# wanxinjin/Learning-from-Sparse-Demonstrations

Measured on AMD Instinct MI355X. Metric: CPDP outer iterations/sec (batch trajectories), higher is better.
Workload: dtype f32; 1 GPU; Quadrotor (JinEnv, initCost_Polynomial, beta time-warp) CPDP, n_grid(horizon) 50 x 4 RK4 steps, batch 4096 per GPU, Nesterov mu 0.9, cold-start OC solve every iteration; BASELINE configs[2]: random initial-guess seeds, one theta and optimizer state per seed, lr 0.01; mode=independent, batch_per_gpu=4096, outer_iters_per_run=50, n_grid=50, steps_per_grid=4, aux_substeps=0, oc_iters_max=7, aux_intervals_accepted_above_rtol=0

## Files before the change

### learning-from-sparse-demonstrations_amd/csrc/cpdp_common.h

```cpp
#pragma once


#include <type_traits>
#if defined(LFSD_EMU)
#include "simt_emu.h"
#define LFSD_LAMBDA_INLINE
#define LFSD_HD
#else
#include <hip/hip_runtime.h>
#define LFSD_DEV __device__ __forceinline__
#define LFSD_HD __host__ __device__
#define LFSD_LAMBDA_INLINE __attribute__((always_inline))
#endif

#ifndef LFSD_COARSE_START
#define LFSD_COARSE_START 1
#endif
#ifndef LFSD_LEAN_TC
#define LFSD_LEAN_TC 2
#endif
#ifndef LFSD_MS
#define LFSD_MS 1
#endif
#ifndef LFSD_COARSE_TIME
#define LFSD_COARSE_TIME 4
#endif
#ifndef LFSD_BW_SMALL
#define LFSD_BW_SMALL 1
#endif
#ifndef LFSD_RIC_PAIR_STAGE
#define LFSD_RIC_PAIR_STAGE 1
#endif

#if defined(LFSD_EMU)
#define LFSD_ROW_FENCE()
#define LFSD_SCHED_FENCE64(T)
#else
#define LFSD_ROW_FENCE() __builtin_amdgcn_sched_barrier(0)
#define LFSD_SCHED_FENCE64(T) do { if constexpr (sizeof(T) == 8) __builtin_amdgcn_sched_barrier(0); } while (0)
#endif

#if defined(LFSD_EMU)
#define LFSD_WAVE_SYNC() __syncthreads()
#else
#define LFSD_WAVE_SYNC()                                            \
  do {                                                              \
    __builtin_amdgcn_fence(__ATOMIC_RELEASE, "workgroup", "local"); \
    __builtin_amdgcn_wave_barrier();                                \
    __builtin_amdgcn_fence(__ATOMIC_ACQUIRE, "workgroup", "local"); \
  } while (0)
#endif

#if defined(LFSD_EMU)
#define LFSD_STAGE_SYNC() __syncthreads()
#else
#define LFSD_STAGE_SYNC() LFSD_WAVE_SYNC()
#endif
#if defined(LFSD_EMU)
#define LFSD_STAGE_SYNC_GEN() __syncthreads()
#else
#define LFSD_STAGE_SYNC_GEN() LFSD_WAVE_SYNC()
#endif

namespace lfsd {

constexpr double kMuUp = 3.1623;
constexpr double kMuDown = 0.31623;
constexpr int kMuHold = 1;
constexpr double kMuStageFracNewton = 0.001;
constexpr double kHamSwitch = 0.3;

constexpr double kCoarseSwitch = 1e-3;
constexpr int kLeanTcS = 1;
constexpr int kLeanTcIters = 3;
constexpr int kLeanTcMin = 12;
constexpr int kLeanTcGrace = 2;
constexpr int kCoarseMinGrid = 40;
constexpr int kMsMinGrid = 40;
constexpr int kCoarseTimeS = 2;
constexpr int kCoarseTimeMin = 20;
constexpr double kCoarseExitMu = 1e-2;
constexpr int kCsAhead = 3;
constexpr int kWideMaxBatch = 1536;

// ... 403 lines not shown
    matmul<n>(A, P, W);
#pragma unroll
    for (int i = 0; i < n * n; ++i) P[i] = -W[i];
#pragma unroll
    for (int i = 0; i < n; ++i) P[i * n + i] += ck[k];
  }
  matmul<n>(A, P, W);
#pragma unroll
  for (int i = 0; i < n * n; ++i) E[i] = -W[i];
#pragma unroll
  for (int i = 0; i < n; ++i) E[i * n + i] += T(1);
  for (int it = 0; it < sq; ++it) {
    matmul<n>(E, P, W);
#pragma unroll
    for (int i = 0; i < n * n; ++i) P[i] = T(0.5) * (P[i] + W[i]);
    matmul<n>(E, E, W);
#pragma unroll
    for (int i = 0; i < n * n; ++i) E[i] = W[i];
  }
  matmul<n>(E, P, W);
#pragma unroll
  for (int i = 0; i < n * n; ++i) P2[i] = T(0.5) * (P[i] + W[i]);
}
template <int Q> constexpr bool sub_ok() { return Q == 1 || Q == 2 || Q == 4; }
#if defined(LFSD_EMU)
template <int Q, typename T> inline T sub_bcast(T v, int k) {
  static_assert(sub_ok<Q>(), "sub-group of 1, 2 or 4 lanes");
  if (Q == 1) return v;
  static T sb[EMU_MAXT];
  const int l = threadIdx.x;
  sb[l] = v;
  __syncthreads();
  const T r = sb[(l & ~(Q - 1)) | k];
  __syncthreads();
  return r;
}
#else
template <int CTRL> LFSD_DEV float dpp_mov(float v) {
  return __builtin_bit_cast(float, __builtin_amdgcn_mov_dpp(__builtin_bit_cast(int, v), CTRL, 0xf, 0xf, true));
}
template <int CTRL> LFSD_DEV double dpp_mov(double v) {
  const unsigned long long u = __builtin_bit_cast(unsigned long long, v);
  const int lo = __builtin_amdgcn_mov_dpp((int)(unsigned)u, CTRL, 0xf, 0xf, true);
  const int hi = __builtin_amdgcn_mov_dpp((int)(unsigned)(u >> 32), CTRL, 0xf, 0xf, true);
  return __builtin_bit_cast(double, ((unsigned long long)(unsigned)hi << 32) | (unsigned long long)(unsigned)lo);
}
template <int Q, typename T> LFSD_DEV T sub_bcast(T v, int k) {
  static_assert(sub_ok<Q>(), "sub-group of 1, 2 or 4 lanes");
  if constexpr (Q == 1) return v;
  else if constexpr (Q == 2) return k == 0 ? dpp_mov<0xA0>(v) : dpp_mov<0xF5>(v);
  else return k == 0 ? dpp_mov<0x00>(v) : (k == 1 ? dpp_mov<0x55>(v) : (k == 2 ? dpp_mov<0xAA>(v) : dpp_mov<0xFF>(v)));
}
#endif
template <int n> constexpr int sub_lanes() { return n <= 1 ? 1 : (n == 2 ? 2 : 4); }
template <int n, int Q, typename T> LFSD_DEV void matmul_rows(const T* Arow, const T* Brow, T* Wrow) {
#pragma unroll
  for (int j = 0; j < n; ++j) Wrow[j] = T(0);
#pragma unroll
  for (int k = 0; k < n; ++k) {
#pragma unroll
    for (int j = 0; j < n; ++j) Wrow[j] += Arow[k] * sub_bcast<Q>(Brow[j], k);
  }
}
template <int n, int Q, typename T> LFSD_DEV void phi1_neg_rows(const T* Mrow, int a, int sq, T sc, T* P, T* P2) {
  T A[n], E[n], W[n];
  const T ck[10] = {T(1), T(1) / T(2), T(1) / T(6), T(1) / T(24), T(1) / T(120), T(1) / T(720), T(1) / T(5040),
                    T(1) / T(40320), T(1) / T(362880), T(1) / T(3628800)};
  constexpr int DEG = PhiDeg<T>::v;
#pragma unroll
  for (int j = 0; j < n; ++j) { A[j] = Mrow[j] * sc; P[j] = (j == a) ? ck[DEG] : T(0); }
#pragma unroll
  for (int k = DEG - 1; k >= 0; --k) {
    matmul_rows<n, Q>(A, P, W);
#pragma unroll
    for (int j = 0; j < n; ++j) P[j] = ((j == a) ? ck[k] : T(0)) - W[j];
  }
  matmul_rows<n, Q>(A, P, W);
#pragma unroll
  for (int j = 0; j < n; ++j) E[j] = ((j == a) ? T(1) : T(0)) - W[j];
  for (int it = 0; it < sq; ++it) {
    matmul_rows<n, Q>(E, P, W);
#pragma unroll
    for (int j = 0; j < n; ++j) P[j] = T(0.5) * (P[j] + W[j]);
    matmul_rows<n, Q>(E, E, W);
#pragma unroll
    for (int j = 0; j < n; ++j) E[j] = W[j];
  }
  matmul_rows<n, Q>(E, P, W);
#pragma unroll
  for (int j = 0; j < n; ++j) P2[j] = T(0.5) * (P[j] + W[j]);
}
template <int n, typename T> LFSD_DEV void matvec(const T* A, const T* v, T* y) {
#pragma unroll
  for (int i = 0; i < n; ++i) {
    T s = T(0);
#pragma unroll
    for (int k = 0; k < n; ++k) s += A[i * n + k] * v[k];
    y[i] = s;
  }
}

}
```

### learning-from-sparse-demonstrations_amd/csrc/cpdp_oc.h

```cpp
#pragma once
#include "cpdp_common.h"

namespace lfsd {

template <typename T> struct OcArgs {
  int batch, n_grid, steps_per_grid, max_iter;
  const T* ini_state;
  const T* horizon;
  const T* auxvar;
  const T* consts;
  int const_stride;
  const T* u_init;
  T* state_grid;
  T* control_grid;
  T* costate_grid;
  T* cost;
  int* iters;
  int* status;
  T* ws;
  long long ws_stride;
  T tol;
  int exact_after;
  int it_start;
  int max_iter_total;
// ... 1252 lines not shown

  LFSD_DEV void costate_sweep_mf(int cur, bool live, T& gnorm) {
    static_assert(G == 16 && NX <= 16 && NEXT <= 1, "16-lane groups, at most one column beyond 16");
    T* ldsME = lds + Lay::LDS_M;  T* ldsLam = lds + Lay::LDS_LAM;  T* ldsRed = lds + Lay::LDS_RED;
    T lam[NX], xk[NX], uk[NU];
    {
      const T* xN = xbp(cur) + N * NX;
#pragma unroll
      for (int i = 0; i < NX; ++i) xk[i] = xN[i];
      M::final_grad(tk(N), xk, e, c, lam);
      if (lane == 0 && live) {
#pragma unroll
        for (int i = 0; i < NX; ++i) lam_out[N * NX + i] = lam[i];
      }
    }
    T gl_max = T(0);
    T m[NX], mq = T(0), me = T(0), mN[NX], mqN = T(0), meN = T(0);
    mf_load_stage(cur, N - 1, m, mq, me, xk, uk);
    for (int k = N - 1; k >= 0; --k) {
      if (NEXT) { if (lane <= NX) ldsME[lane] = me; }
      if (k > 0) { mf_load_stage(cur, k - 1, mN, mqN, meN, xk, uk); LFSD_ISSUE_FENCE(); }
      T gl = mq;
#pragma unroll
      for (int i = 0; i < NX; ++i) gl += m[i] * lam[i];
      if (lane < NX) ldsLam[lane] = gl;
      else if (lane < NCL) gl_max = t_max(gl_max, t_abs(gl));
      __syncthreads();
      if (NEXT) {
        T gl_e = ldsME[NX];
#pragma unroll
        for (int kk = 0; kk < NX; ++kk) gl_e += ldsME[kk] * lam[kk];
        gl_max = t_max(gl_max, (lane == NX) ? t_abs(gl_e) : T(0));
      }
#pragma unroll
      for (int i = 0; i < NX; ++i) lam[i] = ldsLam[i];
      if (lane == 0 && live) {
#pragma unroll
        for (int i = 0; i < NX; ++i) lam_out[k * NX + i] = lam[i];
      }
      __syncthreads();
#pragma unroll
      for (int i = 0; i < NX; ++i) m[i] = mN[i];
      mq = mqN; me = meN;
    }
    ldsRed[lane] = gl_max;
    __syncthreads();
    gnorm = T(0);
#pragma unroll
    for (int a = 0; a < NUL; ++a) gnorm = t_max(gnorm, ldsRed[NX + a]);
    __syncthreads();
  }

  static constexpr int ZC = Lay::ZC, LIVE = Lay::LIVE, LX = NX - Lay::ZC, MS = Lay::MS_ELEMS, LIVEP = Lay::LIVEP;
  LFSD_DEV T rollout_sens_sc(int cur, int nxt, T alpha, bool gains) {
    using V = pk2<T>;
    T x[NX], u[NU], J = T(0);
#pragma unroll
    for (int i = 0; i < NX; ++i) x[i] = x0[i];
    const int c0 = ZC + 2 * lane, c1 = c0 + 1;
    T ubN[NU], xbN[NX], KN[NX * NU], kN[NU];
    auto load_ctl = [&](int k_) LFSD_LAMBDA_INLINE {
      const T* ubk = ubp(cur) + k_ * NU;
#pragma unroll
      for (int a = 0; a < NU; ++a) ubN[a] = ubk[a];
      if (gains) {
        const T* xbk = xbp(cur) + k_ * NX;
        const T* Kk = Kws + (long long)k_ * NX * NU;
        const T* kk = kws + k_ * NU;
#pragma unroll
        for (int i = 0; i < NX; ++i) xbN[i] = xbk[i];
#pragma unroll
        for (int i = 0; i < NX * NU; ++i) KN[i] = Kk[i];
#pragma unroll
        for (int a = 0; a < NU; ++a) kN[a] = kk[a];
      }
    };
    load_ctl(0);
    for (int k = 0; k < N; ++k) {
#pragma unroll
      for (int a = 0; a < NU; ++a) u[a] = ubN[a];
      if (gains) {
#pragma unroll
        for (int a = 0; a < NU; ++a) u[a] += alpha * kN[a];
#pragma unroll
        for (int i = 0; i < NX; ++i) {
          const T dx = x[i] - xbN[i];
#pragma unroll
          for (int a = 0; a < NU; ++a) u[a] += KN[i * NU + a] * dx;
        }
      }
      if (k + 1 < N) { load_ctl(k + 1); LFSD_ISSUE_FENCE(); }
      if (lane == 0) {
#pragma unroll
        for (int i = 0; i < NX; ++i) xbp(nxt)[k * NX + i] = x[i];
#pragma unroll
        for (int a = 0; a < NU; ++a) ubp(nxt)[k * NU + a] = u[a];
      }
      V m[NX], du[NU], mq = V(T(0));
      T q = T(0), qz[ZC ? ZC : 1];
#pragma unroll
      for (int i = 0; i < ZC; ++i) qz[i] = T(0);
#pragma unroll
      for (int i = 0; i < NX; ++i) m[i] = mk2<T>((c0 == i) ? T(1) : T(0), (c1 == i) ? T(1) : T(0));
#pragma unroll
      for (int a = 0; a < NU; ++a) du[a] = mk2<T>((c0 == NX + a) ? T(1) : T(0), (c1 == NX + a) ? T(1) : T(0));
      const T t = tk(k);
// ... 29 lines not shown
      for (int i = 0; i < NX; ++i) m[i] = T(0);
      mq = T(0);
    }
    qzl = (lane >= LX && lane < NX) ? Mk[(NX + 1) * LIVEP + (lane - LX)] : T(0);
    const T* xp = xbp(cur) + k * NX;  const T* up = ubp(cur) + k * NU;
#pragma unroll
    for (int i = 0; i < NX; ++i) xk[i] = xp[i];
#pragma unroll
    for (int a = 0; a < NU; ++a) uk[a] = up[a];
  }
  LFSD_DEV bool backward_sc(int cur, int mode, T mu, bool live, T& gnorm, T& dV1, T& dV2, T& dmin) {
    static_assert(!Lay::sc_ok || (G == 16 && LIVE <= 16 && ZC <= NU && NX <= 16), "structural sweep: 16-lane groups");
    T* ldsV = lds + Lay::LDS_V;  T* ldsK = lds + Lay::LDS_K;
    T* ldsQux = lds + Lay::LDS_QUX;  T* ldsQuu = lds + Lay::LDS_QUU;  T* ldsQu = lds + Lay::LDS_QU;
    T* ldsVx = lds + Lay::LDS_VX;  T* ldsLam = lds + Lay::LDS_LAM;  T* ldsRed = lds + Lay::LDS_RED;
    constexpr bool MM = sizeof(T) == 4;
    constexpr bool VXR = MM;
    T* ldsMl = lds + Lay::LDS_M;
    T* ldsYZ = MM ? lds + Lay::LDS_M : yz64;
    const bool has_v = lane < NX;
    const bool st_zc = lane >= LX && lane < NX;
    const int sv = has_v ? (lane < LX ? ZC + lane : lane - LX) : 0;
    const int zi = st_zc ? lane - LX : 0;
    const bool ctl = lane >= LX && lane < LIVE;
    T Vx[NX], lam[NX], vcol[NX], xk[NX], uk[NU];
    bool ok = true;
    T gl_max = T(0);
    dV1 = T(0); dV2 = T(0); dmin = T(0);
    {
      const T* xN = xbp(cur) + N * NX;
#pragma unroll
      for (int i = 0; i < NX; ++i) xk[i] = xN[i];
      M::final_grad(tk(N), xk, e, c, Vx);
      T ox[NX], oe[NP];
#pragma unroll
      for (int i = 0; i < NX; ++i) { ox[i] = (has_v && sv == i) ? T(1) : T(0); lam[i] = Vx[i]; }
#pragma unroll
      for (int i = 0; i < NP; ++i) oe[i] = T(0);
      M::final_hess_mul(tk(N), xk, e, c, ox, oe, vcol);
      if (lane == 0) {
#pragma unroll
        for (int i = 0; i < NX; ++i) { ldsVx[i] = Vx[i]; ldsLam[i] = lam[i]; }
        if (live) {
#pragma unroll
          for (int i = 0; i < NX; ++i) lam_out[N * NX + i] = lam[i];
        }
      }
      if (!MM && has_v) {
#pragma unroll
        for (int i = 0; i < NX; ++i) ldsV[sv * NX + i] = vcol[i];
      }
    }
    __syncthreads();
    T m[NX], mq = T(0), qzl = T(0);
    sc_load_stage(cur, N - 1, m, mq, qzl, xk, uk);
    for (int k = N - 1; k >= 0; --k) {
      {
#pragma unroll
        for (int a = 0; a < NU; ++a) pin(uk[a]);
#pragma unroll
        for (int i = 0; i < NX; ++i) pin(xk[i]);
        pin(mq); pin(qzl);
      }
      typename std::conditional<MM, f32x16, T[16]>::type acc;
      T yn[NX];
      if constexpr (!MM) {
        if (lane < LIVE) {
#pragma unroll
          for (int i = 0; i < NX; ++i) ldsMl[lane * NX + i] = m[i];
        }
        LFSD_STAGE_SYNC();
        T rowb[2][NX];
#pragma unroll
        for (int kk = 0; kk < NX; ++kk) rowb[0][kk] = ldsV[kk];
#pragma unroll
        for (int r = 0; r < NX + LIVE; ++r) {
          const T* nxt = (r + 1 < NX) ? ldsV + (r + 1) * NX : ldsMl + (r + 1 - NX) * NX;
          if (r + 1 < NX + LIVE) {
#pragma unroll
            for (int kk = 0; kk < NX; ++kk) rowb[(r + 1) & 1][kk] = nxt[kk];
          }
          T sacc = T(0);
          if (r < NX) {
#pragma unroll
            for (int kk = 0; kk < NX; ++kk) sacc += rowb[r & 1][kk] * m[kk];
          } else {
#pragma unroll
            for (int kk = 0; kk < NX; ++kk) sacc += rowb[r & 1][kk] * yn[kk];
          }
          pin(sacc);
          if (r < NX) yn[r] = sacc; else acc[r - NX] = sacc;
          LFSD_ROW_FENCE();
        }
      }
      if constexpr (MM) {
#pragma unroll
      for (int r = 0; r < 16; ++r) acc[r] = 0.f;
#pragma unroll
      for (int kk = 0; kk < NX; ++kk) mfma4b(vcol[kk], m[kk], acc);
      }
      T hx[NX], hu[NU];
      {
        T ox[NX], ou[NU], ls[NX];
        const T HL = (mode == 1) ? T(1) : T(0);
#pragma unroll
        for (int i = 0; i < NX; ++i) { ox[i] = (has_v && sv == i) ? T(1) : T(0); ls[i] = HL * (VXR ? lam[i] : ldsLam[i]); }
#pragma unroll
        for (int a = 0; a < NU; ++a) ou[a] = (lane == LX + a) ? T(1) : T(0);
        M::ham_hess_mul(tk(k), xk, uk, ls, e, c, ox, ou, hx, hu);
      }
      if constexpr (MM) {
        tile_transpose(acc);
#pragma unroll
        for (int s_ = 0; s_ < NX; ++s_) yn[s_] = acc[s_ < ZC ? LX + s_ : s_ - ZC];
      }
      if (lane < LIVE) {
#pragma unroll
        for (int z = 0; z < ZC; ++z) ldsYZ[lane * ZC + z] = yn[z];
      }
      if constexpr (MM) {
#pragma unroll
        for (int r = 0; r < 16; ++r) acc[r] = 0.f;
#pragma unroll
        for (int kk = 0; kk < NX; ++kk) mfma4b(m[kk], yn[kk], acc);
      }
      T Qg = mq, gl = mq;
      if constexpr (VXR) {
#pragma unroll
        for (int i = 0; i < NX; ++i) { Qg += m[i] * Vx[i]; gl += m[i] * lam[i]; }
      } else {
        T vxl[NX], lml[NX];
#pragma unroll
        for (int i = 0; i < NX; ++i) { vxl[i] = ldsVx[i]; lml[i] = ldsLam[i]; }
#pragma unroll
        for (int i = 0; i < NX; ++i) { Qg += m[i] * vxl[i]; gl += m[i] * lml[i]; }
      }
      if constexpr (MM) tile_transpose(acc);
      LFSD_STAGE_SYNC();
      T Qcol[NX], mu_rows[NU], Quxj[NU];
#pragma unroll
      for (int a = 0; a < NU; ++a) mu_rows[a] = acc[LX + a] + dgrid * hu[a];
      T gzv[LIVE];
#pragma unroll
      for (int j = 0; j < LIVE; ++j) gzv[j] = ldsYZ[j * ZC + zi];
      T Vx_z = ldsVx[zi], lam_z = ldsLam[zi];
#pragma unroll
      for (int j = 0; j < LIVE; ++j) pin(gzv[j]);
      pin(Vx_z); pin(lam_z);
#pragma unroll
      for (int j = 0; j < LX; ++j)
        Qcol[ZC + j] = st_zc ? gzv[j] : acc[j] + dgrid * hx[ZC + j];
#pragma unroll
      for (int z = 0; z < ZC; ++z) Qcol[z] = st_zc ? vcol[z] + dgrid * hx[z] : yn[z];
#pragma unroll
      for (int a = 0; a < NU; ++a) Quxj[a] = st_zc ? gzv[LX + a] : mu_rows[a];
      const T Qg_v = st_zc ? qzl + Vx_z : Qg;
      const T gl_v = st_zc ? qzl + lam_z : gl;
      if (has_v) {
#pragma unroll
        for (int a = 0; a < NU; ++a) ldsQux[sv * NU + a] = Quxj[a];
      }
      if (ctl) {
        const int b = lane - LX;
#pragma unroll
        for (int a = 0; a < NU; ++a) ldsQuu[b * NU + a] = mu_rows[a];
        ldsQu[b] = Qg;
        gl_max = t_max(gl_max, t_abs(gl));
      }
      LFSD_STAGE_SYNC();
      T Quu0[NU * NU], Lc[NU * NU], Qu[NU], kff[NU], Kj[NU], t1[NU];
#pragma unroll
      for (int a = 0; a < NU; ++a) {
        Qu[a] = ldsQu[a];
#pragma unroll
        for (int b = 0; b < NU; ++b) Quu0[a * NU + b] = T(0.5) * (ldsQuu[b * NU + a] + ldsQuu[a * NU + b]);
      }
#pragma unroll
      for (int i = 0; i < NU * NU; ++i) Lc[i] = Quu0[i];
#pragma unroll
      for (int a = 0; a < NU; ++a) Lc[a * NU + a] += mu;
      if (ok) ok = chol_factor<NU>(Lc, dmin); else { T dd = T(0); chol_factor<NU>(Lc, dd); }
      {
#pragma unroll
        for (int a = 0; a < NU; ++a) Quu0[a * NU + a] += mu;
      }
#pragma unroll
      for (int a = 0; a < NU; ++a) { kff[a] = -Qu[a]; Kj[a] = -Quxj[a]; }
      chol_solve<NU>(Lc, kff);
      chol_solve<NU>(Lc, Kj);
      T qk[NU];
      matvec<NU>(Quu0, kff, qk);
#pragma unroll
      for (int a = 0; a < NU; ++a) { dV1 += kff[a] * Qu[a]; dV2 += T(0.5) * kff[a] * qk[a]; }
      T Vxj = Qg_v;
#pragma unroll
      for (int a = 0; a < NU; ++a) { Vxj += Kj[a] * (qk[a] + Qu[a]); Vxj += Quxj[a] * kff[a]; }
      if (has_v) {
#pragma unroll
        for (int a = 0; a < NU; ++a) ldsK[sv * NU + a] = Kj[a];
        ldsVx[sv] = Vxj;
        ldsLam[sv] = gl_v;
        if (live) {
          T* Kout = Kws + ((long long)k * NX + sv) * NU;
#pragma unroll
          for (int a = 0; a < NU; ++a) Kout[a] = Kj[a];
        }
      }
      if (lane == 0 && live) {
#pragma unroll
        for (int a = 0; a < NU; ++a) kws[k * NU + a] = kff[a];
      }
      LFSD_STAGE_SYNC();
      matvec<NU>(Quu0, Kj, t1);
#pragma unroll
      for (int a = 0; a < NU; ++a) t1[a] += Quxj[a];
#pragma unroll
      for (int i = 0; i < NX; ++i) {
        T sacc = Qcol[i];
#pragma unroll
        for (int a = 0; a < NU; ++a) { sacc += ldsK[i * NU + a] * t1[a]; sacc += ldsQux[i * NU + a] * Kj[a]; }
        vcol[i] = sacc;
        if (VXR) { Vx[i] = ldsVx[i]; lam[i] = ldsLam[i]; }
      }
      if (lane == 0 && live) {
#pragma unroll
        for (int i = 0; i < NX; ++i) lam_out[k * NX + i] = VXR ? lam[i] : ldsLam[i];
      }
      if (has_v) {
#pragma unroll
        for (int i = 0; i < NX; ++i) ldsV[sv * NX + i] = vcol[i];
      }
      LFSD_STAGE_SYNC();
      {
        T vt[NX];
#pragma unroll
        for (int i = 0; i < NX; ++i) vt[i] = ldsV[i * NX + sv];
#pragma unroll
        for (int i = 0; i < NX; ++i) pin(vt[i]);
#pragma unroll
        for (int i = 0; i < NX; ++i) vcol[i] = has_v ? T(0.5) * (vcol[i] + vt[i]) : T(0);
      }
      LFSD_STAGE_SYNC();
      if (!MM && has_v) {
#pragma unroll
        for (int i = 0; i < NX; ++i) ldsV[sv * NX + i] = vcol[i];
      }
      if (k > 0) sc_load_stage(cur, k - 1, m, mq, qzl, xk, uk);
    }
    ldsRed[lane] = gl_max;
    __syncthreads();
    gnorm = T(0);
#pragma unroll
    for (int a = 0; a < NU; ++a) gnorm = t_max(gnorm, ldsRed[LX + a]);
    __syncthreads();
    if (!t_finite(gnorm) || !t_finite(dV1) || !t_finite(dV2)) ok = false;
    return ok;
  }
  LFSD_DEV void costate_sweep_sc(int cur, bool live, T& gnorm) {
    T* ldsLam = lds + Lay::LDS_LAM;  T* ldsRed = lds + Lay::LDS_RED;
    const bool has_v = lane < NX, st_zc = lane >= LX && lane < NX, ctl = lane >= LX && lane < LIVE;
    const int sv = has_v ? (lane < LX ? ZC + lane : lane - LX) : 0;
    const int zi = st_zc ? lane - LX : 0;
    T lam[NX], xk[NX], uk[NU];
    {
      const T* xN = xbp(cur) + N * NX;
#pragma unroll
      for (int i = 0; i < NX; ++i) xk[i] = xN[i];
      M::final_grad(tk(N), xk, e, c, lam);
      if (lane == 0) {
#pragma unroll
        for (int i = 0; i < NX; ++i) ldsLam[i] = lam[i];
        if (live) {
#pragma unroll
          for (int i = 0; i < NX; ++i) lam_out[N * NX + i] = lam[i];
        }
      }
    }
    __syncthreads();
    T gl_max = T(0);
    T m[NX], mq = T(0), qzl = T(0), mN[NX], mqN = T(0), qzN = T(0);
    sc_load_stage(cur, N - 1, m, mq, qzl, xk, uk);
    for (int k = N - 1; k >= 0; --k) {
      if (k > 0) { sc_load_stage(cur, k - 1, mN, mqN, qzN, xk, uk); LFSD_ISSUE_FENCE(); }
      T gl = mq;
#pragma unroll
      for (int i = 0; i < NX; ++i) gl += m[i] * lam[i];
      if (ctl) gl_max = t_max(gl_max, t_abs(gl));
      T lam_z = ldsLam[zi];
      pin(lam_z);
      const T glz = qzl + lam_z;
      __syncthreads();
      if (has_v) ldsLam[sv] = st_zc ? glz : gl;
      __syncthreads();
#pragma unroll
      for (int i = 0; i < NX; ++i) lam[i] = ldsLam[i];
      if (lane == 0 && live) {
#pragma unroll
        for (int i = 0; i < NX; ++i) lam_out[k * NX + i] = lam[i];
      }
      __syncthreads();
#pragma unroll
      for (int i = 0; i < NX; ++i) m[i] = mN[i];
      mq = mqN; qzl = qzN;
    }
    ldsRed[lane] = gl_max;
    __syncthreads();
    gnorm = T(0);
#pragma unroll
    for (int a = 0; a < NU; ++a) gnorm = t_max(gnorm, ldsRed[LX + a]);
    __syncthreads();
  }

  LFSD_DEV int linesearch(int cur, T J, T dV1, T dV2, T& alpha_out, T& Jmin, bool& flat_full) {
    T* ldsRed = lds + Lay::LDS_RED;
    T alpha = T(0);
    if (lane < NALPHA) { alpha = T(1); for (int i = 0; i < lane; ++i) alpha *= T(0.5); }
    T x[NX], u[NU], Ja = T(0), dummy = T(0);
#pragma unroll
    for (int i = 0; i < NX; ++i) x[i] = x0[i];
    for (int k = 0; k < N; ++k) {
      control(cur, k, x, alpha, true, u);
      T q = T(0);
      const T t = tk(k);
      for (int s = 0; s < S; ++s) rk4_step<false>(t, x, q, u, x, dummy, u);
      Ja += q;
    }
    Ja += M::final_cost(tk(N), x, e, c);
    ldsRed[lane] = Ja;
    __syncthreads();
    int ia = -1;
    Jmin = J;
    T a = T(1);
    alpha_out = T(0);
    const T flat = T(8) * Eps<T>::v() * t_abs(J);
    flat_full = t_finite(ldsRed[0]) && t_abs(ldsRed[0] - J) <= T(64) * Eps<T>::v() * t_abs(J);
    for (int l = 0; l < NALPHA; ++l) {
      const T Jl = ldsRed[l];
      const T expected = -(a * dV1 + a * a * dV2);
      const bool okl = t_finite(Jl) && ((J - Jl) >= T(1e-4) * expected - flat) && (Jl < J);
      if (okl && ia < 0) { ia = l; alpha_out = a; }
      if (t_finite(Jl)) Jmin = t_min(Jmin, Jl);
      a *= T(0.5);
    }
    __syncthreads();
    return ia;
  }
};

template <class M, typename T, bool EXACT, bool BND = false, int W = 1> struct OcWide : OcSolver<M, T, 64, EXACT, BND> {
  using Base = OcSolver<M, T, 64, EXACT, BND>;
  using Lay = OcLayout<M>;
  static constexpr int NX = M::NX, NU = M::NU, NP = M::NP, NXU = NX + NU;
  static constexpr int NAL = 16;
  static constexpr int NW = W, PSTRIDE = 64 * W;
  int wave = 0;
  LFSD_DEV int pitem() const { return W == 1 ? lane : wave * 64 + lane; }
  using Base::lane; using Base::N; using Base::S; using Base::e; using Base::c; using Base::x0; using Base::xb; using Base::ub; using Base::xbp; using Base::ubp; using Base::Mwp;
  using Base::Mws; using Base::Hws; using Base::lds; using Base::xa; using Base::ua; using Base::lam_out; using Base::DT;

  LFSD_DEV T rollout_alphas(int cur, bool gains, T& alpha) {
    alpha = T(0);
    if (lane < NAL) { alpha = T(1); for (int i = 0; i < lane; ++i) alpha *= T(0.5); }
    T x[NX], u[NU], Ja = T(0), dummy = T(0);
// ... 1520 lines not shown
```

### learning-from-sparse-demonstrations_amd/isa_check.py

```python
import re

_FUNC = re.compile(r"^([A-Za-z_][\w$.]*):")
_BLOCK = re.compile(r"^(\.LBB\d+_\d+):")
_EXECZ = re.compile(r"^\s+s_cbranch_execz\s+(\.LBB\d+_\d+)")
_EXECNZ = re.compile(r"^\s+s_cbranch_execnz\s+(\.LBB\d+_\d+)")
_RESTORE = re.compile(r"^(s_or_b64\s+exec,\s*exec,|s_or_saveexec_b64|s_andn2_saveexec_b64|s_xor_b64\s+exec,\s*exec,)")
_SPILL_STORE = re.compile(r"^(v_accvgpr_write_b32\s+a\d+,\s*v\d+|scratch_store_\w+\s.*Folded Spill)")
_SPILL_LOAD = re.compile(r"^(v_accvgpr_read_b32\s+(v\d+),\s*a\d+|scratch_load_(\w+)\s+(v\d+|v\[\d+:\d+\]),.*Folded Reload)")
_VREG = re.compile(r"\bv(\d+)\b|\bv\[(\d+):(\d+)\]")
_EXEC_WRITE = re.compile(r"^s_\w*saveexec|^s_\w+\s+exec\b|^s_mov_b64\s+exec|^s_cmov\w*\s+exec")


def _regs(text):
    out = set()
    for m in _VREG.finditer(text):
        if m.group(1) is not None:
            out.add(int(m.group(1)))
        else:
            out.update(range(int(m.group(2)), int(m.group(3)) + 1))
    return out


def _operands(instr):
    body = instr.split(";")[0]
# ... 31 lines not shown
        else:
            continue
        j, stores, loads, restore_at = i + 1, [], [], -1
        while j < n and (not lines[j].strip() or lines[j].strip().startswith(";") or (label.startswith("behind") and _BLOCK.match(lines[j]))):
            if _BLOCK.match(lines[j]) and _BLOCK.match(lines[j]).group(1) in targets:
                break
            j += 1
        if j < n and _BLOCK.match(lines[j]) and label.startswith("behind"):
            continue
        while j < n:
            t = lines[j].strip()
            if not t or t.startswith(";"):
                j += 1
                continue
            if t.startswith(".L") or t.startswith(("s_branch", "s_cbranch", "s_endpgm", "s_setpc")):
                break
            if _RESTORE.match(t):
                restore_at = j
                break
            if _EXEC_WRITE.match(t):
                break
            if _SPILL_STORE.match(t):
                stores.append((j + 1, t))
            else:
                ml = _SPILL_LOAD.match(t)
                if ml:
                    loads.append((j + 1, t, _regs(ml.group(2) or ml.group(4))))
            j += 1
        if restore_at < 0:
            continue
        for at, t in stores:
            hazards.append({"function": func, "block": label, "line": at, "kind": "spill", "instr": t})
        for at, t, regs in loads:
            pending, k = set(regs), restore_at + 1
            bad = False
            while k < n and pending:
                u = lines[k].strip()
                if not u or u.startswith(";"):
                    k += 1
                    continue
                if u.startswith(".L") or u.startswith(("s_branch", "s_cbranch", "s_endpgm", "s_setpc")):
                    break
                w, r = _operands(u)
                if r & pending:
                    bad = True
                    break
                pending -= w
                k += 1
            if bad:
                hazards.append({"function": func, "block": label, "line": at, "kind": "reload", "instr": t})
    return hazards


def summary(asm_text):
    targets = set(m.group(1) for m in (_EXECZ.match(ln) for ln in asm_text.split("\n")) if m)
    nfunc = sum(1 for ln in asm_text.split("\n") if ln.startswith(".Lfunc_end"))
    return {"functions": nfunc, "join_blocks": len(targets)}
```

### learning-from-sparse-demonstrations_amd/runtime.py

```python
import ctypes
import os
import shutil
import subprocess

import torch

PKG_DIR = os.path.dirname(os.path.abspath(__file__))
CSRC_DIR = os.path.join(PKG_DIR, "csrc")
GEN_DIR = os.path.join(CSRC_DIR, "gen")
BUILD_DIR = os.path.join(CSRC_DIR, "build")
INCLUDE_DIR = os.path.join(os.path.dirname(PKG_DIR), "include")

LFSD_F32, LFSD_F64 = 0, 1
STATUS = {1: "converged", 2: "stalled", 3: "maxiter", 4: "failed"}
OPT_METHODS = {"Vanilla": 0, "Nesterov": 1, "Adam": 2, "Nadam": 3, "AMSGrad": 4, "LM": 5}
MAPPINGS = {"auto": 0, "lockstep": 1, "wide": 2}


class LfsdError(RuntimeError):
    pass


class _ModelInfo(ctypes.Structure):
    _fields_ = [("abi_version", ctypes.c_int), ("n_state", ctypes.c_int), ("n_control", ctypes.c_int),
# ... 18 lines not shown
            return cand
    raise LfsdError("hipcc not found: the HIP model library cannot be built")


def library_path(model_hash):
    return os.path.join(BUILD_DIR, "liblfsd_%s.so" % model_hash)


def header_path(model_hash):
    return os.path.join(GEN_DIR, "%s.h" % model_hash)


def write_header(spec, force=False):
    from . import codegen
    os.makedirs(GEN_DIR, exist_ok=True)
    hp = header_path(spec.hash())
    if force or not os.path.exists(hp):
        src = codegen.emit_header(spec)
        tmp = hp + ".tmp%d" % os.getpid()
        with open(tmp, "w") as f:
            f.write(src)
        os.replace(tmp, hp)
    return hp


def _hipcc_flags(spec, extra=()):
    g = lanes_for(spec.n, spec.m, spec.p)
    return [find_hipcc(), "-x", "hip", "--offload-arch=gfx950", "-std=c++17", "-O3", "-fPIC",
            "-fno-signed-zeros", "-fvisibility=hidden",
            "-DLFSD_G=%d" % g, '-DLFSD_MODEL_HEADER="gen/%s.h"' % spec.hash(), "-I" + CSRC_DIR] + list(extra)


TUNED_CAPI = ()
TUNED_RICCATI = ()
TUNED_CUBIC = ()
UNITS = ("capi", "riccati", "cubic")


def hipcc_commands(spec, out, extra=(), extra_capi=TUNED_CAPI, extra_riccati=TUNED_RICCATI, extra_cubic=TUNED_CUBIC):
    flags = _hipcc_flags(spec, extra) + ["-fno-slp-vectorize"]
    o1, o2, o3 = out + ".capi.o", out + ".riccati.o", out + ".cubic.o"
    return ([flags + ["-c", "-DLFSD_SPLIT_RICCATI", os.path.join(CSRC_DIR, "lfsd_capi.cpp"), "-o", o1] + list(extra_capi),
             flags + ["-c", os.path.join(CSRC_DIR, "lfsd_riccati.cpp"), "-o", o2] + list(extra_riccati),
             flags + ["-c", os.path.join(CSRC_DIR, "lfsd_cubic.cpp"), "-o", o3] + list(extra_cubic),
             [find_hipcc(), "--offload-arch=gfx950", "-shared", "-fPIC", o1, o2, o3, "-o", out]], [o1, o2, o3])


KERNEL_SOURCES = ("cpdp_kernels.h", "cpdp_common.h", "cpdp_oc.h", "cpdp_aux.h", "cpdp_opt.h", "cpdp_rows.h", "cpdp_spline.h", "cpdp_sample.h", "cpdp_lm.h", "cpdp_groups.h", "cpdp_aux_sweeps.inc", "lfsd_capi.cpp",
                  "lfsd_internal.h", "lfsd_riccati.inc", "lfsd_riccati.cpp", "lfsd_cubic.inc", "lfsd_cubic.cpp")


SCHEDULE_ALTERNATES = ((), ("-mllvm", "-amdgpu-sched-strategy=max-ilp"), ("-mllvm", "-amdgpu-sched-strategy=max-memory-clause"),
                       ("-mllvm", "-amdgpu-use-amdgpu-trackers"), ("-mllvm", "-greedy-reverse-local-assignment"))
ISA_CHECK_VERSION = 3


def isa_record_path(lib_path):
    return lib_path + ".isa.json"


def isa_record_clean(lib_path):
    import json
    try:
        rec = json.load(open(isa_record_path(lib_path)))
    except (OSError, ValueError):
        return False
    units = rec.get("units", {})
    return rec.get("isa_check") == ISA_CHECK_VERSION and set(units) == set(UNITS) and all(u.get("hazards") == 0 for u in units.values()) \
        and rec.get("sha256") == _sha256(lib_path)


def _sha256(path):
    import hashlib
    h = hashlib.sha256()
    with open(path, "rb") as f:
        for chunk in iter(lambda: f.read(1 << 20), b""):
            h.update(chunk)
    return h.hexdigest()


def _checked_build(spec, out, extra=(), verbose=False, what="model"):
    import json, shutil, tempfile
    from . import isa_check
    os.makedirs(BUILD_DIR, exist_ok=True)
    work = tempfile.mkdtemp(prefix="obj%d_" % os.getpid(), dir=BUILD_DIR)
    try:
        tmp = os.path.join(work, "lib.so")
        record = {"isa_check": ISA_CHECK_VERSION, "units": {}}
        objs = []
        for ui, unit in enumerate(UNITS):
            tuned = (TUNED_CAPI, TUNED_RICCATI, TUNED_CUBIC)[ui]
            tried, built = [], False
            for alt in SCHEDULE_ALTERNATES:
                kw = {"extra_" + unit: tuple(tuned) + tuple(alt)}
                cmds, obj_paths = hipcc_commands(spec, tmp, list(extra), **kw)
                cmd = cmds[ui] + ["-save-temps=obj"]
                if verbose:
                    print(" ".join(cmd))
                for f in os.listdir(work):
                    if f.endswith(".s"):
                        os.remove(os.path.join(work, f))
                r = subprocess.run(cmd, cwd=CSRC_DIR, capture_output=True, text=True)
                if r.returncode != 0:
                    if alt:
                        tried.append({"flags": list(alt), "error": r.stderr[-300:]})
                        continue
                    raise LfsdError("hipcc failed for %s %s:\n%s\n%s" % (what, spec.name, r.stdout[-4000:], r.stderr[-4000:]))
                asm = [f for f in os.listdir(work) if f.endswith("gfx950.s")]
                if len(asm) != 1:
                    raise LfsdError("no device assembly to check for %s %s (%s): %s" % (what, spec.name, unit, sorted(os.listdir(work))))
                text = open(os.path.join(work, asm[0])).read()
                hz = isa_check.find_exec_hazards(text)
                if hz:
                    tried.append({"flags": list(alt), "hazards": len(hz), "first": hz[0]})
                    if verbose:
                        print("isa_check: %d spill(s) before an exec restore in %s (%s, flags %s): %s" % (len(hz), spec.name, unit, list(alt), hz[0]))
                    continue
                record["units"][unit] = dict(isa_check.summary(text), flags=list(tuned) + list(alt), hazards=0, rejected=tried)
                objs.append(obj_paths[ui])
                built = True
                break
            if not built:
                raise LfsdError("every build of %s %s (%s) has VGPR spills before an exec restore (lfsd_amd/isa_check.py): %s"
                                % (what, spec.name, unit, tried))
        link = hipcc_commands(spec, tmp, list(extra))[0][-1]
        r = subprocess.run(link, cwd=CSRC_DIR, capture_output=True, text=True)
        if r.returncode != 0:
            raise LfsdError("link failed for %s %s:\n%s" % (what, spec.name, r.stderr[-3000:]))
        record["sha256"] = _sha256(tmp)
        with open(isa_record_path(out) + ".tmp%d" % os.getpid(), "w") as f:
            json.dump(record, f, indent=1, sort_keys=True, default=str)
        os.replace(tmp, out)
        os.replace(isa_record_path(out) + ".tmp%d" % os.getpid(), isa_record_path(out))
        return record
    finally:
        shutil.rmtree(work, ignore_errors=True)


def build_library(spec, force=False, verbose=False):
    os.makedirs(BUILD_DIR, exist_ok=True)
    out = library_path(spec.hash())
    write_header(spec, force=force)
    deps = [header_path(spec.hash()), os.path.join(INCLUDE_DIR, "lfsd_cpdp.h")] + \
        [os.path.join(CSRC_DIR, f) for f in KERNEL_SOURCES]
    if not force and os.path.exists(out) and all(os.path.getmtime(out) >= os.path.getmtime(d) for d in deps) and isa_record_clean(out):
        return out
    _checked_build(spec, out, verbose=verbose)
    return out


def variant_library_path(spec, tag):
    return os.path.join(BUILD_DIR, "ab_%s_%s.so" % (spec.hash(), tag))


def build_variant_library(spec, tag, flags):
    write_header(spec)
    out = variant_library_path(spec, tag)
    deps = [header_path(spec.hash())] + [os.path.join(CSRC_DIR, f) for f in KERNEL_SOURCES]
    if os.path.exists(out) and all(os.path.getmtime(out) >= os.path.getmtime(p) for p in deps) and isa_record_clean(out):
        return out
    _checked_build(spec, out, extra=list(flags), what="variant %s of model" % tag)
    return out


PLAIN_SCHEDULE = ("-DLFSD_LEAN_TC=1", "-DLFSD_COARSE_START=0", "-DLFSD_COARSE_TIME=1", "-DLFSD_MS=0")
GPU_TIER_VARIANTS = (("quadrotor", 50, "nocoarse", ("-DLFSD_COARSE_START=0",)),
                     ("quadrotor", 50, "plain", PLAIN_SCHEDULE), ("cartpole", 40, "plain", PLAIN_SCHEDULE),
                     ("rocket", 40, "plain", PLAIN_SCHEDULE), ("robotarm", 50, "plain", PLAIN_SCHEDULE),
                     ("quadrotor", 50, "ricpair0", ("-DLFSD_RIC_PAIR_STAGE=0",)))


def build_gpu_tier_variants(verbose=False):
    from concurrent.futures import ThreadPoolExecutor
    from . import models
    built = {}
    with ThreadPoolExecutor(max_workers=max(1, min(4, (os.cpu_count() or 2) // 2))) as pool:
        futs = {}
        for kind, n_grid, tag, flags in GPU_TIER_VARIANTS:
            oc = models.ZOO[kind](n_grid=n_grid)[0]
            futs[(kind, tag)] = pool.submit(build_variant_library, oc.model_spec(), tag, flags)
        for (kind, tag), fut in futs.items():
            try:
                built[(kind, tag)] = fut.result()
                if verbose:
                    print("variant", kind, tag, built[(kind, tag)])
            except Exception as exc:
                print("WARNING: test variant %s/%s not built: %s" % (kind, tag, str(exc)[:300]))
    return built


_DT = {torch.float32: LFSD_F32, torch.float64: LFSD_F64}


class ModelLibrary:

    EXPORTS = ("lfsd_get_model_info", "lfsd_interface_dim", "lfsd_const_default", "lfsd_coc_workspace_bytes", "lfsd_coc_solve",
               "lfsd_aux_solve", "lfsd_aux_riccati", "lfsd_aux_forward", "lfsd_optimizer_step", "lfsd_lookahead",
               "lfsd_stop_compact", "lfsd_gather_rows", "lfsd_scatter_rows", "lfsd_grid_curvature", "lfsd_aux_solve_cubic",
               "lfsd_aux_riccati_cubic", "lfsd_aux_forward_cubic", "lfsd_sample_grid", "lfsd_waypoint_vjp",
               "lfsd_optimizer_step_rows", "lfsd_lookahead_rows", "lfsd_trace_append", "lfsd_normal_matrix", "lfsd_lm_step",
               "lfsd_group_reduce")

    def __init__(self, path):
        if not os.path.exists(path):
            raise LfsdError("model library %s does not exist (build it with __graft_entry__.build() or "
                            "COCSys.compile())" % path)
        self.path = path
        self.lib = ctypes.CDLL(path)
        for sym in self.EXPORTS:
            if not hasattr(self.lib, sym):
                raise LfsdError("%s does not export %s" % (path, sym))
        L = self.lib
        vp, ci, cd = ctypes.c_void_p, ctypes.c_int, ctypes.c_double
        L.lfsd_get_model_info.argtypes = [ctypes.POINTER(_ModelInfo)]
        L.lfsd_const_default.argtypes = [ci]
        L.lfsd_const_default.restype = cd
        L.lfsd_coc_workspace_bytes.argtypes = [ci, ci, ci, ci, ci, ci]
        L.lfsd_coc_workspace_bytes.restype = ctypes.c_size_t
        L.lfsd_coc_solve.argtypes = [ci, ci, ci, ci, vp, vp, vp, vp, ci, vp, vp, vp, vp, vp, vp, cd, vp, vp, vp, vp, vp, vp, ci, cd, ci,
                                     ci, vp, ctypes.c_size_t, vp]
        L.lfsd_aux_solve.argtypes = [ci, ci, ci, vp, vp, vp, ci, vp, vp, vp, vp, ci, ci, vp, vp, vp, vp, vp, vp, vp,
                                     ci, cd, vp, vp, ci, vp]
# ... 526 lines not shown
```

Baseline: 960,200 trajectory outer-iterations/s.

## Replace LDS exchanges in the OC backward Riccati sweep with DPP row broadcasts

In the sensitivity/costate backward sweep, when a group is one 16-lane row and T is f32, per-stage LDS writes, stage syncs and reads of Quu, Qu, K, Qux, Vx and lambda are replaced by DPP row_newbcast broadcasts and inline v_fmac_f32_dpp asm. The final gradient-norm reduction also moves from LDS to row broadcasts. The aim is to remove LDS traffic and barriers on the serial per-stage critical path. In exchange it adds hand-written DPP asm with an s_nop settle, and an ISA checker that rejects builds placing DPP reads too close to a writer, which could force a fallback schedule.

Result: faster. 987,900 trajectory outer-iterations/s (median of 6 runs) (+2.9%).

```diff
diff --git a/learning-from-sparse-demonstrations_amd/csrc/cpdp_common.h b/learning-from-sparse-demonstrations_amd/csrc/cpdp_common.h
--- a/learning-from-sparse-demonstrations_amd/csrc/cpdp_common.h
+++ b/learning-from-sparse-demonstrations_amd/csrc/cpdp_common.h
@@ -2,6 +2,7 @@
 
 
 #include <type_traits>
+#include <utility>
 #if defined(LFSD_EMU)
 #include "simt_emu.h"
 #define LFSD_LAMBDA_INLINE
@@ -30,6 +31,9 @@
 #endif
 #ifndef LFSD_RIC_PAIR_STAGE
 #define LFSD_RIC_PAIR_STAGE 1
+#endif
+#ifndef LFSD_OC_DPP_XCHG
+#define LFSD_OC_DPP_XCHG 1
 #endif
 
 #if defined(LFSD_EMU)
@@ -539,6 +543,48 @@
   else return k == 0 ? dpp_mov<0x00>(v) : (k == 1 ? dpp_mov<0x55>(v) : (k == 2 ? dpp_mov<0xAA>(v) : dpp_mov<0xFF>(v)));
 }
 #endif
+constexpr bool row_xchg_ok(int lanes) { return lanes == 16; }
+#if defined(LFSD_EMU)
+template <typename T> inline T row_bcast(T v, int k) {
+  static T sb[EMU_MAXT];
+  const int l = threadIdx.x;
+  sb[l] = v;
+  __syncthreads();
+  const T r = sb[(l & ~15) | k];
+  __syncthreads();
+  return r;
+}
+#else
+LFSD_DEV float row_bcast(float v, int k) {
+  switch (k) {
+    case 0: return dpp_mov<0x150>(v);   case 1: return dpp_mov<0x151>(v);   case 2: return dpp_mov<0x152>(v);   case 3: return dpp_mov<0x153>(v);
+    case 4: return dpp_mov<0x154>(v);   case 5: return dpp_mov<0x155>(v);   case 6: return dpp_mov<0x156>(v);   case 7: return dpp_mov<0x157>(v);
+    case 8: return dpp_mov<0x158>(v);   case 9: return dpp_mov<0x159>(v);   case 10: return dpp_mov<0x15A>(v);  case 11: return dpp_mov<0x15B>(v);
+    case 12: return dpp_mov<0x15C>(v);  case 13: return dpp_mov<0x15D>(v);  case 14: return dpp_mov<0x15E>(v);  default: return dpp_mov<0x15F>(v);
+  }
+}
+#endif
+#if defined(LFSD_EMU)
+inline void dpp_settle() {}
+template <int K> inline void fmac2_row_bcast(float& acc, float a, float wa, float b, float wb) {
+  acc += row_bcast(a, K) * wa;
+  acc += row_bcast(b, K) * wb;
+}
+#else
+LFSD_DEV void dpp_settle() { asm volatile("s_nop 4"); }
+template <int K> LFSD_DEV void fmac2_row_bcast(float& acc, float a, float wa, float b, float wb) {
+  static_assert(K >= 0 && K < 16, "lane of the row");
+  asm volatile("v_fmac_f32_dpp %0, %1, %2 row_newbcast:%5 row_mask:0xf bank_mask:0xf bound_ctrl:1\n\t"
+               "v_fmac_f32_dpp %0, %3, %4 row_newbcast:%5 row_mask:0xf bank_mask:0xf bound_ctrl:1"
+               : "+v"(acc) : "v"(a), "v"(wa), "v"(b), "v"(wb), "n"(K));
+}
+#endif
+template <typename T> LFSD_DEV T row_max(T v, int first, int n) {
+  T r = T(0);
+#pragma unroll
+  for (int a = 0; a < n; ++a) r = t_max(r, row_bcast(v, first + a));
+  return r;
+}
 template <int n> constexpr int sub_lanes() { return n <= 1 ? 1 : (n == 2 ? 2 : 4); }
 template <int n, int Q, typename T> LFSD_DEV void matmul_rows(const T* Arow, const T* Brow, T* Wrow) {
 #pragma unroll
diff --git a/learning-from-sparse-demonstrations_amd/csrc/cpdp_oc.h b/learning-from-sparse-demonstrations_amd/csrc/cpdp_oc.h
--- a/learning-from-sparse-demonstrations_amd/csrc/cpdp_oc.h
+++ b/learning-from-sparse-demonstrations_amd/csrc/cpdp_oc.h
@@ -1328,6 +1328,16 @@
   }
 
   static constexpr int ZC = Lay::ZC, LIVE = Lay::LIVE, LX = NX - Lay::ZC, MS = Lay::MS_ELEMS, LIVEP = Lay::LIVEP;
+  static constexpr bool XD = (LFSD_OC_DPP_XCHG != 0) && sizeof(T) == 4 && row_xchg_ok(G);
+  static constexpr int sc_lane(int i) { return i < ZC ? LX + i : i - ZC; }
+  template <int I> LFSD_DEV void sc_vrow(T& sacc, const T* Kj, const T* t1, const T* Quxj) const {
+#pragma unroll
+    for (int a = 0; a < NU; ++a) fmac2_row_bcast<sc_lane(I)>(sacc, Kj[a], t1[a], Quxj[a], Kj[a]);
+  }
+  template <int... I> LFSD_DEV void sc_vrows(T* vcol, const T* Kj, const T* t1, const T* Quxj, std::integer_sequence<int, I...>) const {
+    dpp_settle();
+    (sc_vrow<I>(vcol[I], Kj, t1, Quxj), ...);
+  }
   LFSD_DEV T rollout_sens_sc(int cur, int nxt, T alpha, bool gains) {
     using V = pk2<T>;
     T x[NX], u[NU], J = T(0);
@@ -1463,6 +1473,8 @@
       }
     }
     __syncthreads();
+    T Vx_own = T(0), lam_own = T(0);
+    if constexpr (XD) { Vx_own = ldsVx[sv]; lam_own = ldsLam[sv]; }
     T m[NX], mq = T(0), qzl = T(0);
     sc_load_stage(cur, N - 1, m, mq, qzl, xk, uk);
     for (int k = N - 1; k >= 0; --k) {
@@ -1554,10 +1566,11 @@
       T gzv[LIVE];
 #pragma unroll
       for (int j = 0; j < LIVE; ++j) gzv[j] = ldsYZ[j * ZC + zi];
-      T Vx_z = ldsVx[zi], lam_z = ldsLam[zi];
+      T Vx_z, lam_z;
+      if constexpr (XD) { Vx_z = Vx_own; lam_z = lam_own; } else { Vx_z = ldsVx[zi]; lam_z = ldsLam[zi]; }
 #pragma unroll
       for (int j = 0; j < LIVE; ++j) pin(gzv[j]);
-      pin(Vx_z); pin(lam_z);
+      if constexpr (!XD) { pin(Vx_z); pin(lam_z); }
 #pragma unroll
       for (int j = 0; j < LX; ++j)
         Qcol[ZC + j] = st_zc ? gzv[j] : acc[j] + dgrid * hx[ZC + j];
@@ -1567,24 +1580,40 @@
       for (int a = 0; a < NU; ++a) Quxj[a] = st_zc ? gzv[LX + a] : mu_rows[a];
       const T Qg_v = st_zc ? qzl + Vx_z : Qg;
       const T gl_v = st_zc ? qzl + lam_z : gl;
-      if (has_v) {
-#pragma unroll
-        for (int a = 0; a < NU; ++a) ldsQux[sv * NU + a] = Quxj[a];
-      }
-      if (ctl) {
-        const int b = lane - LX;
-#pragma unroll
-        for (int a = 0; a < NU; ++a) ldsQuu[b * NU + a] = mu_rows[a];
-        ldsQu[b] = Qg;
-        gl_max = t_max(gl_max, t_abs(gl));
-      }
-      LFSD_STAGE_SYNC();
       T Quu0[NU * NU], Lc[NU * NU], Qu[NU], kff[NU], Kj[NU], t1[NU];
-#pragma unroll
-      for (int a = 0; a < NU; ++a) {
-        Qu[a] = ldsQu[a];
-#pragma unroll
-        for (int b = 0; b < NU; ++b) Quu0[a * NU + b] = T(0.5) * (ldsQuu[b * NU + a] + ldsQuu[a * NU + b]);
+      if constexpr (XD) {
+        if (ctl) gl_max = t_max(gl_max, t_abs(gl));
+        T Qr[NU * NU];
+#pragma unroll
+        for (int b = 0; b < NU; ++b) {
+#pragma unroll
+          for (int a = 0; a < NU; ++a) Qr[b * NU + a] = row_bcast(mu_rows[a], LX + b);
+          Qu[b] = row_bcast(Qg, LX + b);
+        }
+#pragma unroll
+        for (int a = 0; a < NU; ++a) {
+#pragma unroll
+          for (int b = 0; b < NU; ++b) Quu0[a * NU + b] = T(0.5) * (Qr[b * NU + a] + Qr[a * NU + b]);
+        }
+      } else {
+        if (has_v) {
+#pragma unroll
+          for (int a = 0; a < NU; ++a) ldsQux[sv * NU + a] = Quxj[a];
+        }
+        if (ctl) {
+          const int b = lane - LX;
+#pragma unroll
+          for (int a = 0; a < NU; ++a) ldsQuu[b * NU + a] = mu_rows[a];
+          ldsQu[b] = Qg;
+          gl_max = t_max(gl_max, t_abs(gl));
+        }
+        LFSD_STAGE_SYNC();
+#pragma unroll
+        for (int a = 0; a < NU; ++a) {
+          Qu[a] = ldsQu[a];
+#pragma unroll
+          for (int b = 0; b < NU; ++b) Quu0[a * NU + b] = T(0.5) * (ldsQuu[b * NU + a] + ldsQuu[a * NU + b]);
+        }
       }
 #pragma unroll
       for (int i = 0; i < NU * NU; ++i) Lc[i] = Quu0[i];
@@ -1607,10 +1636,12 @@
 #pragma unroll
       for (int a = 0; a < NU; ++a) { Vxj += Kj[a] * (qk[a] + Qu[a]); Vxj += Quxj[a] * kff[a]; }
       if (has_v) {
-#pragma unroll
-        for (int a = 0; a < NU; ++a) ldsK[sv * NU + a] = Kj[a];
-        ldsVx[sv] = Vxj;
-        ldsLam[sv] = gl_v;
+        if constexpr (!XD) {
+#pragma unroll
+          for (int a = 0; a < NU; ++a) ldsK[sv * NU + a] = Kj[a];
+          ldsVx[sv] = Vxj;
+          ldsLam[sv] = gl_v;
+        }
         if (live) {
           T* Kout = Kws + ((long long)k * NX + sv) * NU;
 #pragma unroll
@@ -1621,17 +1652,25 @@
 #pragma unroll
         for (int a = 0; a < NU; ++a) kws[k * NU + a] = kff[a];
       }
-      LFSD_STAGE_SYNC();
+      if constexpr (!XD) LFSD_STAGE_SYNC();
       matvec<NU>(Quu0, Kj, t1);
 #pragma unroll
       for (int a = 0; a < NU; ++a) t1[a] += Quxj[a];
 #pragma unroll
       for (int i = 0; i < NX; ++i) {
         T sacc = Qcol[i];
-#pragma unroll
-        for (int a = 0; a < NU; ++a) { sacc += ldsK[i * NU + a] * t1[a]; sacc += ldsQux[i * NU + a] * Kj[a]; }
+        if constexpr (XD) {
+          Vx[i] = row_bcast(Vxj, sc_lane(i)); lam[i] = row_bcast(gl_v, sc_lane(i));
+        } else {
+#pragma unroll
+          for (int a = 0; a < NU; ++a) { sacc += ldsK[i * NU + a] * t1[a]; sacc += ldsQux[i * NU + a] * Kj[a]; }
+          if (VXR) { Vx[i] = ldsVx[i]; lam[i] = ldsLam[i]; }
+        }
         vcol[i] = sacc;
-        if (VXR) { Vx[i] = ldsVx[i]; lam[i] = ldsLam[i]; }
+      }
+      if constexpr (XD) {
+        sc_vrows(vcol, Kj, t1, Quxj, std::make_integer_sequence<int, NX>());
+        Vx_own = Vxj; lam_own = gl_v;
       }
       if (lane == 0 && live) {
 #pragma unroll
@@ -1658,12 +1697,16 @@
       }
       if (k > 0) sc_load_stage(cur, k - 1, m, mq, qzl, xk, uk);
     }
-    ldsRed[lane] = gl_max;
-    __syncthreads();
-    gnorm = T(0);
-#pragma unroll
-    for (int a = 0; a < NU; ++a) gnorm = t_max(gnorm, ldsRed[LX + a]);
-    __syncthreads();
+    if constexpr (XD) {
+      gnorm = row_max(gl_max, LX, NU);
+    } else {
+      ldsRed[lane] = gl_max;
+      __syncthreads();
+      gnorm = T(0);
+#pragma unroll
+      for (int a = 0; a < NU; ++a) gnorm = t_max(gnorm, ldsRed[LX + a]);
+      __syncthreads();
+    }
     if (!t_finite(gnorm) || !t_finite(dV1) || !t_finite(dV2)) ok = false;
     return ok;
   }
@@ -1689,6 +1732,8 @@
     }
     __syncthreads();
     T gl_max = T(0);
+    T lam_own = T(0);
+    if constexpr (XD) lam_own = ldsLam[sv];
     T m[NX], mq = T(0), qzl = T(0), mN[NX], mqN = T(0), qzN = T(0);
     sc_load_stage(cur, N - 1, m, mq, qzl, xk, uk);
     for (int k = N - 1; k >= 0; --k) {
@@ -1697,29 +1742,39 @@
 #pragma unroll
       for (int i = 0; i < NX; ++i) gl += m[i] * lam[i];
       if (ctl) gl_max = t_max(gl_max, t_abs(gl));
-      T lam_z = ldsLam[zi];
-      pin(lam_z);
-      const T glz = qzl + lam_z;
-      __syncthreads();
-      if (has_v) ldsLam[sv] = st_zc ? glz : gl;
-      __syncthreads();
-#pragma unroll
-      for (int i = 0; i < NX; ++i) lam[i] = ldsLam[i];
+      if constexpr (XD) {
+        lam_own = st_zc ? qzl + lam_own : gl;
+#pragma unroll
+        for (int i = 0; i < NX; ++i) lam[i] = row_bcast(lam_own, sc_lane(i));
+      } else {
+        T lam_z = ldsLam[zi];
+        pin(lam_z);
+        const T glz = qzl + lam_z;
+        __syncthreads();
+        if (has_v) ldsLam[sv] = st_zc ? glz : gl;
+        __syncthreads();
+#pragma unroll
+        for (int i = 0; i < NX; ++i) lam[i] = ldsLam[i];
+      }
       if (lane == 0 && live) {
 #pragma unroll
         for (int i = 0; i < NX; ++i) lam_out[k * NX + i] = lam[i];
       }
-      __syncthreads();
+      if constexpr (!XD) __syncthreads();
 #pragma unroll
       for (int i = 0; i < NX; ++i) m[i] = mN[i];
       mq = mqN; qzl = qzN;
     }
-    ldsRed[lane] = gl_max;
-    __syncthreads();
-    gnorm = T(0);
-#pragma unroll
-    for (int a = 0; a < NU; ++a) gnorm = t_max(gnorm, ldsRed[LX + a]);
-    __syncthreads();
+    if constexpr (XD) {
+      gnorm = row_max(gl_max, LX, NU);
+    } else {
+      ldsRed[lane] = gl_max;
+      __syncthreads();
+      gnorm = T(0);
+#pragma unroll
+      for (int a = 0; a < NU; ++a) gnorm = t_max(gnorm, ldsRed[LX + a]);
+      __syncthreads();
+    }
   }
 
   LFSD_DEV int linesearch(int cur, T J, T dV1, T dV2, T& alpha_out, T& Jmin, bool& flat_full) {
diff --git a/learning-from-sparse-demonstrations_amd/isa_check.py b/learning-from-sparse-demonstrations_amd/isa_check.py
--- a/learning-from-sparse-demonstrations_amd/isa_check.py
+++ b/learning-from-sparse-demonstrations_amd/isa_check.py
@@ -107,7 +107,124 @@
     return hazards
 
 
+_DPP = re.compile(r"^(v_\w+_dpp)\s+(.*?)\s+(?:quad_perm:|row_\w+|wave_\w+|bank_mask:|bound_ctrl:|fi:)")
+_LABEL = re.compile(r"^(\.L[\w$.]+):")
+_BRANCH = re.compile(r"^s_c?branch\w*\s+(\.L[\w$.]+)")
+_END = ("s_branch", "s_endpgm", "s_setpc_b64")
+_TRANS = ("v_exp_", "v_log_", "v_rcp_", "v_rsq_", "v_sqrt_", "v_sin_", "v_cos_")
+_NOP = re.compile(r"^s_nop\s+(\d+)")
+_MFMA_SHAPE = re.compile(r"_(\d+)x\d+x?\d*")
+DPP_SRC0_WAIT, DPP_EXEC_WAIT, TRANS_WAIT = 2, 5, 1
+
+
+def _mfma_wait(op):
+    m = _MFMA_SHAPE.search(op)
+    edge = int(m.group(1)) if m else 32
+    return 5 if edge <= 4 else (11 if edge <= 16 else 19)
+
+
+def _vector_writes(instr):
+    parts = instr.split(";")[0].split(None, 1)
+    if len(parts) < 2 or not parts[0].startswith("v_") or parts[0].startswith("v_cmp"):
+        return set()
+    ops = parts[1].split(",")
+    if parts[0].startswith("v_swap") or (parts[0].startswith("v_permlane") and "swap" in parts[0]):
+        return _regs(",".join(ops[:2]))
+    return _regs(ops[0])
+
+
+def _writes_exec_vector(instr):
+    op = instr.split(None, 1)[0]
+    return op.startswith("v_cmpx") or (op.startswith(("v_readlane", "v_readfirstlane")) and re.match(r"^\S+\s+exec", instr) is not None)
+
+
+def find_dpp_hazards(asm_text):
+    ins, line_of, func_of, labelled, first = [], [], [], [], set()
+    branches = {}
+    func, pending, entry = None, [], True
+    for i, ln in enumerate(asm_text.split("\n")):
+        t = ln.strip()
+        if not t or t.startswith(";"):
+            continue
+        m = _FUNC.match(ln)
+        if m and not ln.startswith(".L"):
+            func, pending, entry = m.group(1), [], True
+            continue
+        m = _LABEL.match(t)
+        if m:
+            pending.append(m.group(1))
+            continue
+        if t.startswith(".") or t.endswith(":"):
+            continue
+        t = t.split(";")[0].strip()
+        if not t:
+            continue
+        k = len(ins)
+        ins.append(t)
+        line_of.append(i + 1)
+        func_of.append(func)
+        labelled.append(pending)
+        if entry:
+            first.add(k)
+        pending, entry = [], False
+        m = _BRANCH.match(t)
+        if m:
+            branches.setdefault(m.group(1), []).append(k)
+
+    def preds(p):
+        out = []
+        if p not in first and p > 0 and not ins[p - 1].startswith(_END):
+            out.append(p - 1)
+        for lab in labelled[p]:
+            out.extend(branches.get(lab, ()))
+        return out
+
+    def writer_within(d, window, is_writer):
+        stack, seen = [(d, window)], {}
+        while stack:
+            p, w = stack.pop()
+            for q in preds(p):
+                if is_writer(ins[q]):
+                    return q
+                nop = _NOP.match(ins[q])
+                w2 = w - (int(nop.group(1)) + 1 if nop else 1)
+                if w2 > 0 and seen.get(q, 0) < w2:
+                    seen[q] = w2
+                    stack.append((q, w2))
+        return None
+
+    hazards = []
+    for d, t in enumerate(ins):
+        m = _DPP.match(t)
+        if not m:
+            continue
+        ops = m.group(2).split(",")
+        src0 = _regs(ops[1]) if len(ops) > 1 else set()
+        reads = _regs(",".join(ops[1:])) | (_regs(ops[0]) if "mac" in m.group(1) else set())
+        rules = [("dpp-src0", DPP_SRC0_WAIT, lambda u: bool(_vector_writes(u) & src0)),
+                 ("dpp-exec", DPP_EXEC_WAIT, _writes_exec_vector),
+                 ("dpp-trans", TRANS_WAIT, lambda u: u.startswith(_TRANS) and bool(_vector_writes(u) & reads))]
+        for edge_wait in (5, 11, 19):
+            rules.append(("dpp-mfma", edge_wait, lambda u, e=edge_wait: u.startswith(("v_mfma", "v_smfmac")) and _mfma_wait(u.split(None, 1)[0]) >= e
+                          and bool(_vector_writes(u) & reads)))
+        for kind, window, is_writer in rules:
+            q = writer_within(d, window, is_writer)
+            if q is not None:
+                hazards.append({"function": func_of[d], "block": (labelled[d] or ["line %d" % line_of[d]])[0], "line": line_of[d], "kind": kind,
+                                "instr": t, "writer": ins[q], "writer_line": line_of[q]})
+                break
+    return hazards
+
+
+def find_hazards(asm_text):
+    return find_exec_hazards(asm_text) + find_dpp_hazards(asm_text)
+
+
 def summary(asm_text):
     targets = set(m.group(1) for m in (_EXECZ.match(ln) for ln in asm_text.split("\n")) if m)
     nfunc = sum(1 for ln in asm_text.split("\n") if ln.startswith(".Lfunc_end"))
     return {"functions": nfunc, "join_blocks": len(targets)}
+
+
+def dpp_count(asm_text):
+    return sum(1 for ln in asm_text.split("\n") if _DPP.match(ln.strip()))
diff --git a/learning-from-sparse-demonstrations_amd/runtime.py b/learning-from-sparse-demonstrations_amd/runtime.py
--- a/learning-from-sparse-demonstrations_amd/runtime.py
+++ b/learning-from-sparse-demonstrations_amd/runtime.py
@@ -94,7 +94,7 @@
 
 SCHEDULE_ALTERNATES = ((), ("-mllvm", "-amdgpu-sched-strategy=max-ilp"), ("-mllvm", "-amdgpu-sched-strategy=max-memory-clause"),
                        ("-mllvm", "-amdgpu-use-amdgpu-trackers"), ("-mllvm", "-greedy-reverse-local-assignment"))
-ISA_CHECK_VERSION = 3
+ISA_CHECK_VERSION = 4
 
 
 def isa_record_path(lib_path):
@@ -152,18 +152,18 @@
                 if len(asm) != 1:
                     raise LfsdError("no device assembly to check for %s %s (%s): %s" % (what, spec.name, unit, sorted(os.listdir(work))))
                 text = open(os.path.join(work, asm[0])).read()
-                hz = isa_check.find_exec_hazards(text)
+                hz = isa_check.find_exec_hazards(text) + isa_check.find_dpp_hazards(text)
                 if hz:
                     tried.append({"flags": list(alt), "hazards": len(hz), "first": hz[0]})
                     if verbose:
-                        print("isa_check: %d spill(s) before an exec restore in %s (%s, flags %s): %s" % (len(hz), spec.name, unit, list(alt), hz[0]))
+                        print("isa_check: %d spill(s) before an exec restore / DPP instruction(s) too close to a writer in %s (%s, flags %s): %s" % (len(hz), spec.name, unit, list(alt), hz[0]))
                     continue
-                record["units"][unit] = dict(isa_check.summary(text), flags=list(tuned) + list(alt), hazards=0, rejected=tried)
+                record["units"][unit] = dict(isa_check.summary(text), dpp=isa_check.dpp_count(text), flags=list(tuned) + list(alt), hazards=0, rejected=tried)
                 objs.append(obj_paths[ui])
                 built = True
                 break
             if not built:
-                raise LfsdError("every build of %s %s (%s) has VGPR spills before an exec restore (lfsd_amd/isa_check.py): %s"
+                raise LfsdError("every build of %s %s (%s) has VGPR spills before an exec restore or a DPP instruction too close to a writer (lfsd_amd/isa_check.py): %s"
                                 % (what, spec.name, unit, tried))
         link = hipcc_commands(spec, tmp, list(extra))[0][-1]
         r = subprocess.run(link, cwd=CSRC_DIR, capture_output=True, text=True)
@@ -209,7 +209,8 @@
 GPU_TIER_VARIANTS = (("quadrotor", 50, "nocoarse", ("-DLFSD_COARSE_START=0",)),
                      ("quadrotor", 50, "plain", PLAIN_SCHEDULE), ("cartpole", 40, "plain", PLAIN_SCHEDULE),
                      ("rocket", 40, "plain", PLAIN_SCHEDULE), ("robotarm", 50, "plain", PLAIN_SCHEDULE),
-                     ("quadrotor", 50, "ricpair0", ("-DLFSD_RIC_PAIR_STAGE=0",)))
+                     ("quadrotor", 50, "ricpair0", ("-DLFSD_RIC_PAIR_STAGE=0",)),
+                     ("quadrotor", 50, "ocdpp0", ("-DLFSD_OC_DPP_XCHG=0",)), ("rocket", 40, "ocdpp0", ("-DLFSD_OC_DPP_XCHG=0",)))
 
 
 def build_gpu_tier_variants(verbose=False):
```
